# ipo-lab/lqp_py

Hardware: AMD Instinct MI355X
Metric: QPs/sec forward+backward, batch=128 dz=500 tol=1e-5 (higher is better)
Workload: dtype f32; 1 GPU; BASELINE configs[2]: batch=128/GPU dz=500 m=1 box+equality QP, ADMM forward + fixed-point backward, eps 1e-5, scale+adaptive_rho defaults; global_batch=128, seeds=10 batches, seeds 0..9 per rank, cycled, iters=60, checks=4, launch_mode=3, sync=False, linsolve=spd, loop_workgroups_per_qp=2, parallelism=batch-sharded x1, rccl_world_size=1

## Files before the change

### include/lqp_amd.h

```cpp
#ifndef LQP_AMD_H
#define LQP_AMD_H

#include <stddef.h>
#include <stdint.h>

#ifdef __cplusplus
extern "C" {
#endif

#define LQP_ABI_VERSION 14

enum { LQP_F32 = 0, LQP_F64 = 1 };

enum {
    LQP_OK = 0,
    LQP_ERR_INVALID = 1,
    LQP_ERR_WORKSPACE = 2,
    LQP_ERR_SINGULAR = 3,
    LQP_ERR_HIP = 4,
    LQP_ERR_TIMEOUT = 5,
    LQP_ERR_UNSUPPORTED = 6,
    LQP_ERR_NOT_SPD = 7
};

typedef struct lqp_boxqp_ctrl {
    int32_t max_iters;
    int32_t check_solved;
    int32_t adaptive_rho;
    int32_t adaptive_rho_iter;
    int32_t adaptive_rho_max_iter;
    int32_t scale;
    int32_t any_lb;
    int32_t any_ub;
    int32_t rho_mode;
    int32_t beta_mode;
    int32_t launch_mode;
    int32_t reserved;
    int32_t linsolve;
    int32_t reserved2;
    double eps_abs;
    double eps_rel;
    double rho_value;
    double rho_min;
// ... 7 lines not shown
    const void* bound_flags_in;
    void* host_report;
} lqp_boxqp_ctrl;

typedef struct lqp_boxqp_stats {
    int32_t iters;
    int32_t n_factor;
    int32_t n_solve;
    int32_t n_check;
    int32_t rho_updated;
    int32_t fail_index;
    int32_t n_launch;
    int32_t mode_used;
    int32_t linsolve_used;
    int32_t factor_launches;
    int32_t loop_workgroups;
    int32_t any_lb;
    int32_t any_ub;
    int32_t loop_kind;
} lqp_boxqp_stats;

int lqp_abi_version(void);
const char* lqp_status_string(int status);

void lqp_profile_enable(int on);
void lqp_profile_reset(void);
int lqp_profile_classes(void);
const char* lqp_profile_class_name(int cls);
int lqp_profile_get(double* total_ms, long long* launches, int n);
void lqp_debug_set_lu_counters(void* device_buf);
int lqp_debug_spin(void* stream, int blocks, int usec, int lds_bytes);
int lqp_debug_xcd(void* stream, int blocks, void* out_dev);
int lqp_debug_lu_inverse(void* stream, int dtype, int B, int N, const void* packed, void* X_out);

size_t lqp_boxqp_forward_workspace_bytes(int dtype, int B, int n, int m);
int lqp_boxqp_forward_layout(int dtype, int B, int n, int m, size_t* status_offset, size_t* status_bytes,
                             size_t* info_offset, size_t* info_bytes);
int lqp_boxqp_forward(void* stream, int dtype, int B, int n, int m,
                      const void* Q, const void* p, const void* A, const void* b,
                      const void* lb, const void* ub,
                      const lqp_boxqp_ctrl* ctrl, const void* rho_in,
                      void* x, void* z, void* u, void* lams, void* nus, void* rho_out,
                      lqp_boxqp_stats* stats,
                      void* workspace, size_t workspace_bytes);

int lqp_boxqp_forward_finish(void* stream, int B, int max_iters, int check_solved, const void* host_report,
                             lqp_boxqp_stats* stats);

size_t lqp_boxqp_unroll_backward_workspace_bytes(int B, int n, int m, int iters);
int lqp_boxqp_unroll_backward(void* stream, int B, int n, int m, const void* fwd_workspace, size_t fwd_workspace_bytes,
                              int iters, const void* dl_dx, void* dQs, void* dps, void* dAs, void* dbs, void* dlbs,
                              void* dubs, void* drho, void* dD, void* scratch, size_t scratch_bytes);

size_t lqp_boxqp_unroll_backward_lu_workspace_bytes(int dtype, int B, int n, int m, int iters);
int lqp_boxqp_unroll_backward_lu(void* stream, int dtype, int B, int n, int m, const void* fwd_workspace, size_t fwd_workspace_bytes,
                                 int iters, const void* dl_dx, void* dQs, void* dps, void* dAs, void* dbs, void* dlbs, void* dubs,
                                 void* drho, void* dD, void* scratch, size_t scratch_bytes);

size_t lqp_boxqp_unroll_tape_workspace_bytes(int dtype, int B, int n, int m, int iters);
int lqp_boxqp_unroll_tape_segment(void* stream, int dtype, int B, int n, int m, const void* fwd_workspace, size_t fwd_workspace_bytes,
                                  int iters, int k0, int k1, int mode, const void* packed_buf, const void* rho, void* state, int inj_k,
                                  const void* inj, const void* dl_dx, void* dps, void* dlbs, void* dubs, void* drho, void* dD,
                                  void* scratch, size_t scratch_bytes, void** z_rows, void** u_rows, void** x_rows);
int lqp_boxqp_unroll_tape_finish(void* stream, int dtype, int B, int n, int m, int iters, void* dQs, void* dAs, void* dbs, void* scratch,
                                 size_t scratch_bytes);

// ... 79 lines not shown
```

### lqp_py_amd/_lib.py

```python
import ctypes
import os
import subprocess
import threading

import numpy

import torch

HERE = os.path.dirname(os.path.abspath(__file__))
CSRC = os.path.join(HERE, "csrc")
LIB_PATH = os.environ.get("LQP_LIB", os.path.join(CSRC, "liblqp_amd.so"))
SOURCES = ["lqp_amd.hip", "lqp_unroll.hpp", "lqp_boxqp.hpp", "lqp_loop_split.hpp", "lqp_loop_small.hpp", "lqp_lu.hpp", "lqp_lu_big.hpp", "lqp_lu2.hpp", "lqp_lu_wide.hpp", "lqp_dense.hpp", "lqp_trsv.hpp", "lqp_spd.hpp", "lqp_f16x2.hpp", "lqp_common.hpp"]

LQP_F32, LQP_F64 = 0, 1
ABI_VERSION = 14
STATUS = {0: "ok", 1: "invalid argument", 2: "workspace too small", 3: "singular", 4: "HIP error",
          5: "grid barrier timeout", 6: "unsupported size (n + m <= 4096 in float32, 2048 in float64)", 7: "matrix outside the symmetric x-update"}

c_void_p, c_int, c_size_t, c_double = ctypes.c_void_p, ctypes.c_int, ctypes.c_size_t, ctypes.c_double


CHECK_HOOK = ctypes.CFUNCTYPE(ctypes.c_int, ctypes.c_void_p, ctypes.c_void_p, ctypes.c_void_p, ctypes.c_int)


class BoxQPCtrl(ctypes.Structure):
    _fields_ = [(k, ctypes.c_int32) for k in (
        "max_iters", "check_solved", "adaptive_rho", "adaptive_rho_iter", "adaptive_rho_max_iter", "scale",
        "any_lb", "any_ub", "rho_mode", "beta_mode", "launch_mode", "reserved", "linsolve", "reserved2")] + [
        (k, ctypes.c_double) for k in (
            "eps_abs", "eps_rel", "rho_value", "rho_min", "rho_max", "adaptive_rho_tol",
            "adaptive_rho_threshold", "beta_value")] + [
        ("beta_in", ctypes.c_void_p), ("check_hook", CHECK_HOOK), ("check_hook_user", ctypes.c_void_p),
        ("bound_flags_in", ctypes.c_void_p), ("host_report", ctypes.c_void_p)]


class BoxQPStats(ctypes.Structure):
    _fields_ = [(k, ctypes.c_int32) for k in (
        "iters", "n_factor", "n_solve", "n_check", "rho_updated", "fail_index", "n_launch", "mode_used", "linsolve_used",
        "factor_launches", "loop_workgroups", "any_lb", "any_ub", "loop_kind")]


_P = c_void_p
SYMBOLS = {
    "lqp_abi_version": (c_int, []),
    "lqp_status_string": (ctypes.c_char_p, [c_int]),
    "lqp_profile_enable": (None, [c_int]),
    "lqp_profile_reset": (None, []),
    "lqp_profile_classes": (c_int, []),
    "lqp_profile_class_name": (ctypes.c_char_p, [c_int]),
    "lqp_profile_get": (c_int, [ctypes.POINTER(c_double), ctypes.POINTER(ctypes.c_longlong), c_int]),
    "lqp_debug_set_lu_counters": (None, [_P]),
    "lqp_debug_spin": (c_int, [_P, c_int, c_int, c_int]),
    "lqp_debug_xcd": (c_int, [_P, c_int, _P]),
    "lqp_debug_lu_inverse": (c_int, [_P, c_int, c_int, c_int, _P, _P]),
    "lqp_boxqp_forward_workspace_bytes": (c_size_t, [c_int] * 4),
    "lqp_boxqp_forward": (c_int, [_P, c_int, c_int, c_int, c_int, _P, _P, _P, _P, _P, _P,
                                  ctypes.POINTER(BoxQPCtrl), _P, _P, _P, _P, _P, _P, _P,
                                  ctypes.POINTER(BoxQPStats), _P, c_size_t]),
    "lqp_boxqp_forward_finish": (c_int, [_P, c_int, c_int, c_int, _P, ctypes.POINTER(BoxQPStats)]),
    "lqp_boxqp_forward_layout": (c_int, [c_int] * 4 + [ctypes.POINTER(c_size_t)] * 4),
    "lqp_boxqp_unroll_backward_workspace_bytes": (c_size_t, [c_int] * 4),
    "lqp_boxqp_unroll_backward": (c_int, [_P, c_int, c_int, c_int, _P, c_size_t, c_int] + [_P] * 10 + [c_size_t]),
    "lqp_boxqp_unroll_backward_lu_workspace_bytes": (c_size_t, [c_int] * 5),
    "lqp_boxqp_unroll_backward_lu": (c_int, [_P, c_int, c_int, c_int, c_int, _P, c_size_t, c_int] + [_P] * 10 + [c_size_t]),
    "lqp_boxqp_unroll_tape_workspace_bytes": (c_size_t, [c_int] * 5),
    "lqp_boxqp_unroll_tape_segment": (c_int, [_P, c_int, c_int, c_int, c_int, _P, c_size_t, c_int, c_int, c_int, c_int, _P, _P, _P, c_int]
                                      + [_P] * 8 + [c_size_t] + [_P] * 3),
    "lqp_boxqp_unroll_tape_finish": (c_int, [_P, c_int, c_int, c_int, c_int, c_int, _P, _P, _P, _P, c_size_t]),
    "lqp_unroll_scale_colmax": (c_int, [_P, c_int, c_int, _P, _P, _P, _P]),
    "lqp_unroll_scale_grad_slabs": (c_int, [c_int, c_int]),
    "lqp_unroll_scale_grad": (c_int, [_P, c_int, c_int, _P, _P, _P, _P, _P, c_int]),
    "lqp_unroll_scale_vectors": (c_int, [_P, c_int, c_int, c_int, c_int, c_int, c_int, c_double] + [_P] * 13 + [c_int] + [_P] * 7),
    "lqp_unroll_scale_scatter": (c_int, [_P, c_int, c_int, _P, _P, _P, _P, _P, _P]),
    "lqp_boxqp_last_residuals": (c_int, [_P, c_int, c_int, c_int, c_int, _P, c_size_t, _P, _P]),
    "lqp_boxqp_problem_iters": (c_int, [_P, c_int, c_int, c_int, c_int, _P, c_size_t, _P]),
    "lqp_boxqp_check_trace": (c_int, [_P, c_int, c_int, c_int, c_int, _P, c_size_t, c_int, _P]),
    "lqp_boxqp_backward_fp_workspace_bytes": (c_size_t, [c_int] * 4),
    "lqp_boxqp_backward_fp_prefactor": (c_int, [_P, c_int, c_int, c_int, c_int] + [_P] * 6 + [_P, c_size_t, c_int, _P]),
    "lqp_boxqp_backward_fp": (c_int, [_P, c_int, c_int, c_int, c_int] + [_P] * 9 + [c_int, c_double, _P] + [_P] * 6 +
                              [ctypes.POINTER(ctypes.c_int32), _P, c_size_t, c_int, _P]),
    "lqp_boxqp_backward_kkt": (c_int, [_P, c_int, c_int, c_int, c_int] + [_P] * 8 + [_P] * 6 +
                               [ctypes.POINTER(ctypes.c_int32), _P, c_size_t, c_int, _P]),
    "lqp_lu_factor_workspace_bytes": (c_size_t, [c_int] * 3),
    "lqp_lu_factor_batched": (c_int, [_P, c_int, c_int, c_int, _P, _P, _P, _P, c_size_t]),
    "lqp_lu_solve_workspace_bytes": (c_size_t, [c_int] * 3),
    "lqp_lu_solve_batched": (c_int, [_P, c_int, c_int, c_int, c_int, _P, _P, _P, _P, c_size_t]),
    "lqp_lu_packed_bytes": (c_size_t, [c_int] * 3),
# ... 315 lines not shown
```

### lqp_py_amd/csrc/lqp_amd.hip

```cpp
#include "../../include/lqp_amd.h"
#include "lqp_boxqp.hpp"
#include "lqp_unroll.hpp"
#ifdef LQP_SPLIT_BUILD
#include "split/lqp_extern.inc"
#endif

#include <cstdio>
#include <cstdlib>
#include <cstring>
#include <algorithm>
#include <atomic>
#include <chrono>
#include <mutex>
#include <vector>
#include <string>
#include <type_traits>
#include <unordered_map>
#include <unordered_set>

using namespace lqp;

namespace {

constexpr int kRing = 2048;
// ... 1740 lines not shown
    smem[threadIdx.x] = 0;
    const unsigned long long t0 = __builtin_amdgcn_s_memrealtime();
    while (__builtin_amdgcn_s_memrealtime() - t0 < ticks) __builtin_amdgcn_s_sleep(32);
}
int lqp_debug_spin(void* stream, int blocks, int usec, int lds_bytes) {
    if (blocks < 1 || usec < 0 || usec > 2000000 || lds_bytes < 512) return LQP_ERR_INVALID;
    const int rc = ensure_lds((const void*)k_debug_spin, lds_bytes);
    if (rc) return rc;
    hipLaunchKernelGGL(k_debug_spin, dim3(blocks), dim3(512), lds_bytes, (hipStream_t)stream, (unsigned long long)usec * 100ull);
    return last_error();
}

__global__ __launch_bounds__(512) void k_debug_xcd(int* __restrict__ out) {
    if (threadIdx.x == 0) out[blockIdx.x] = (int)my_xcd();
}
int lqp_debug_xcd(void* stream, int blocks, void* out_dev) {
    if (blocks < 1 || !out_dev) return LQP_ERR_INVALID;
    hipLaunchKernelGGL(k_debug_xcd, dim3(blocks), dim3(512), 0, (hipStream_t)stream, (int*)out_dev);
    return last_error();
}

int lqp_debug_lu_inverse(void* stream, int dtype, int B, int N, const void* packed_buf, void* X_out) {
    if (bad_dims(dtype, B, N, 0) || !packed_buf || !X_out || N > (dtype == LQP_F32 ? 2048 : 1024)) return LQP_ERR_INVALID;
    const int K = round_up(N, LQP_NB) / LQP_NB;
    return by_dtype(dtype, [&](auto t) {
        using T = decltype(t);
        int* dest; T* packed;
        carve_packed<T>((void*)packed_buf, B, N, dest, packed);
        return launch_lu_inverse<T>((hipStream_t)stream, B, N, packed, packed_blocks(K) * LQP_BLK, dest, K * LQP_NB, (T*)X_out,
                                    (size_t)N * N, N, nullptr);
    });
}

int lqp_profile_classes(void) { return PC_COUNT; }

const char* lqp_profile_class_name(int c) {
    static const char* names[PC_COUNT] = {"fwd_setup", "lu_factor", "pack", "admm_loop", "rho_update", "fwd_epilogue",
                                          "bwd_build", "packed_solve", "bwd_epilogue", "misc", "admm_loop_tail",
                                          "spd_inverse", "eq_correct", "bwd_cholesky", "unroll_backward", "unroll_scaling"};
    return (c >= 0 && c < PC_COUNT) ? names[c] : "?";
}

int lqp_profile_get(double* total_ms, long long* launches, int n) {
    std::lock_guard<std::mutex> lock(g_prof_mutex);
    for (auto& r : g_prof_recs) {
        if (hipEventSynchronize(r.b) != hipSuccess) return LQP_ERR_HIP;
        float ms = 0.f;
        if (hipEventElapsedTime(&ms, r.a, r.b) != hipSuccess) return LQP_ERR_HIP;
        g_prof_ms[r.cls] += ms;
        g_prof_n[r.cls] += 1;
        (void)hipEventDestroy(r.a); (void)hipEventDestroy(r.b);
    }
    g_prof_recs.clear();
    for (int i = 0; i < n && i < PC_COUNT; ++i) { total_ms[i] = g_prof_ms[i]; launches[i] = g_prof_n[i]; }
    return LQP_OK;
}

const char* lqp_status_string(int s) {
    switch (s) {
        case LQP_OK: return "ok";
        case LQP_ERR_INVALID: return "invalid argument";
        case LQP_ERR_WORKSPACE: return "workspace too small";
        case LQP_ERR_SINGULAR: return "singular matrix (exactly zero pivot)";
        case LQP_ERR_HIP: return "HIP runtime error";
        case LQP_ERR_TIMEOUT: return "in-kernel grid barrier timed out";
        case LQP_ERR_UNSUPPORTED: return "size not supported by this build (n + m <= 4096 in float32, 2048 in float64)";
// ... 391 lines not shown
```

### lqp_py_amd/csrc/lqp_boxqp.hpp

```cpp
#pragma once
#include <type_traits>
#include "lqp_common.hpp"
#include "lqp_lu.hpp"
#include "lqp_lu_big.hpp"
#include "lqp_lu2.hpp"
#include "lqp_lu_wide.hpp"
#include "lqp_trsv.hpp"
#include "lqp_spd.hpp"

namespace lqp {

enum { ST_DONE = 0, ST_FINAL_ITER = 1, ST_GATE = 2, ST_NFACTOR = 3, ST_RHO_UPDATED = 4,
       ST_TIMEOUT = 5, ST_NCHECK = 6, ST_NOTSPD = 7,
       ST_VOTE = 8,
       ST_ANY_LB = 12, ST_ANY_UB = 13,
       ST_RESUME = 14,
       ST_NDONE = 15,
       ST_WORDS = 16 };
enum { PS_DONE = 0, PS_FINAL = 1, PS_RESUME = 2, PS_NFACTOR = 3, PS_WORDS = 4 };
enum { RP_LB = 1, RP_UB = 2, RP_TIMEOUT = 4, RP_NOTSPD = 8 };
enum { CT_NOTOPT = 0, CT_ARRIVE = 1, CT_WANTS = 2, CT_TRIG = 3, CT_WORDS = 4 };
template <typename T>
__device__ __forceinline__ void trace_check(unsigned int* __restrict__ vtrace, const int it, const int check_solved, const int ring,
                                            const T pri, const T dua) {
// ... 2035 lines not shown
    extern __shared__ __attribute__((aligned(32))) char smem[];
    const int b = blockIdx.x, n = P.n, m = P.m, Np = P.Np;
    const int tid = threadIdx.x, lane = tid & 63, w = tid >> 6;
    const int Kmax = round_up(n, LQP_NB) / LQP_NB, Npm = Kmax * LQP_NB;
    const int nf = P.nred[b] - m;
    const int Kb = round_up(nf, LQP_NB) / LQP_NB, Nb = Kb * LQP_NB;
    float* Ls = P.packed + (size_t)b * sym_blocks(Kmax) * LQP_BLK;
    const float* AF = P.M + (size_t)b * Np * Np;
    float* rhs = P.rhs + (size_t)b * Np;
    unsigned long long dt0 = P.dbg ? clock64() : 0;
    if (Kb > 0 && P.phase != 2) {
        if (Kb <= P.la_maxk) wg_chol_factor_la<F16>(Ls, Kb, P.info + b, smem, P.dbg ? P.dbg + (size_t)b * 8 : nullptr);
        else if (Kb <= SPD_MAXK) wg_chol_factor(Ls, Kb, P.info + b, smem);
        else wg_chol_factor_big(Ls, Kb, P.info + b, smem);
    }
    if (P.host_report && (P.early_report || P.phase == 1) && !P.reported) {
        __syncthreads();
        if (tid == 0)
            __hip_atomic_store(P.host_report + b, __hip_atomic_load(P.info + b, __ATOMIC_RELAXED, __HIP_MEMORY_SCOPE_AGENT),
                               __ATOMIC_RELAXED, __HIP_MEMORY_SCOPE_SYSTEM);
    }
    if (P.phase == 1) return;
    __syncthreads();
    if (P.dbg && tid == 0) { const unsigned long long t = clock64(); P.dbg[(size_t)b * 8 + 0] = t - dt0; dt0 = t; P.dbg[(size_t)b * 8 + 3] = Kb; }
    constexpr int NR = NRV == 4 ? 4 : 2;
    float* acc = (float*)smem;
    float* u0 = acc + (size_t)NR * Npm;
    float* G = u0 + Npm;
    float* t = G + (size_t)m * Npm;
    float* part = t + NR * 64;
    float* S = part + NR * LQP_NW * 64;
    float* wv = S + m * m;
    float* dn = wv + m;
    if (P.phase == 2) {
        const float* g = P.g + (size_t)b * n;
        const int* fidx = P.fidx + (size_t)b * n;
        const float* bs_ = P.bsc ? P.bsc + (size_t)b * Np : nullptr;
        for (int e = tid; e < Nb; e += LQP_NT) u0[e] = e < nf ? -g[fidx[e]] * (bs_ ? bs_[e] : 1.f) : 0.f;
    } else {
        for (int e = tid; e < Nb; e += LQP_NT) u0[e] = rhs[e];
    }
    for (int q = 0; q < m; ++q)
        for (int e = tid; e < Nb; e += LQP_NT) G[(size_t)q * Npm + e] = AF[(size_t)q * Npm + e];
    __syncthreads();
    if (Kb > 0)
        for (int c0 = 0; c0 < 1 + m; c0 += NR)
            wg_chol_solve_n<NR>(Ls, Kb, u0 + (size_t)c0 * Npm, Npm, (1 + m - c0) < NR ? (1 + m - c0) : NR, acc, t, part,
                                (P.dbg && P.la_maxk == 0) ? P.dbg + (size_t)b * 8 : nullptr);
    if (P.dbg && tid == 0) { const unsigned long long t = clock64(); P.dbg[(size_t)b * 8 + 1] = t - dt0; dt0 = t; }
    if (m > 0) {
        for (int e = w; e < m * m + m; e += LQP_NW) {
            const int q = e < m * m ? e / m : e - m * m;
            const float* rv = e < m * m ? G + (size_t)(e - q * m) * Npm : u0;
            float a = 0.f;
            for (int i = lane; i < nf; i += 64) a += AF[(size_t)q * Npm + i] * rv[i];
            a = wave_sum(a);
            if (lane == 0) {
                if (e < m * m) S[e] = a - ((e / m == e % m) ? 1e-8f : 0.f);
                else wv[q] = a;
            }
        }
        __syncthreads();
        {
            const int rr = tid / (m + 1), jj = tid - rr * (m + 1);
            const bool mine = tid < m * (m + 1);
            int* pivrow = (int*)dn;
            for (int c = 0; c < m; ++c) {
                if (tid == 0) {
                    int pr = c;
                    float best = tabs(S[c * m + c]);
                    for (int r2 = c + 1; r2 < m; ++r2) if (tabs(S[r2 * m + c]) > best) { best = tabs(S[r2 * m + c]); pr = r2; }
                    const bool skip = !(best > 0.f);
                    if (skip && P.info[b] == 0) P.info[b] = nf + c + 1;
                    pivrow[0] = pr; pivrow[1] = skip ? 1 : 0;
                }
                __syncthreads();
                const int pr = pivrow[0];
                const bool skip = pivrow[1] != 0;
                float* const rowc = jj < m ? S + c * m + jj : wv + c;
                float* const rowp = jj < m ? S + pr * m + jj : wv + pr;
                float* const rowr = jj < m ? S + rr * m + jj : wv + rr;
                if (!skip && pr != c && tid <= m) {
                    const float tmp = *rowc; *rowc = *rowp; *rowp = tmp;
                }
                __syncthreads();
                const float inv = skip ? 0.f : 1.f / S[c * m + c];
                const float f = (mine && !skip) ? S[rr * m + c] : 0.f;
                __syncthreads();
                if (!skip && tid <= m) *rowc *= inv;
                __syncthreads();
                if (mine && !skip && rr != c) *rowr -= f * *rowc;
                __syncthreads();
            }
            for (int q = tid; q < m; q += LQP_NT) dn[q] = wv[q];
        }
        __syncthreads();
    }
    for (int a = tid; a < nf; a += LQP_NT) {
        float d = u0[a];
        for (int q = 0; q < m; ++q) d -= G[(size_t)q * Npm + a] * dn[q];
        rhs[a] = P.bsc ? d * P.bsc[(size_t)b * Np + a] : d;
    }
    for (int q = tid; q < m; q += LQP_NT) rhs[nf + q] = dn[q];
    if (P.dbg && tid == 0) P.dbg[(size_t)b * 8 + 2] = clock64() - dt0;
}

template <typename T>
__global__ __launch_bounds__(LQP_NT) void k_bwd_residual(const BwdParams<T> P) {
    extern __shared__ __attribute__((aligned(32))) char smem[];
    const int b = blockIdx.x, n = P.n, m = P.m, Np = P.Np;
    const int tid = threadIdx.x, lane = tid & 63, w = tid >> 6;
    T* dvf = (T*)smem;
    T* dn = dvf + round_up(n, 8);
    int* fl = (int*)(dn + round_up(m > 0 ? m : 1, 8));
    const int nf = P.nred[b] - m;
    const T* d = P.rhs + (size_t)b * Np;
    T* r = P.rhs2 + (size_t)b * Np;
    const T* Q = P.Q + (size_t)b * n * n;
    const T* A = P.A ? P.A + (size_t)b * m * n : nullptr;
    const T* g = P.g + (size_t)b * n;
    for (int i = tid; i < n; i += LQP_NT) dvf[i] = T(0);
    for (int a = tid; a < nf; a += LQP_NT) fl[a] = P.fidx[(size_t)b * n + a];
    for (int q = tid; q < m; q += LQP_NT) dn[q] = d[nf + q];
    __syncthreads();
    for (int a = tid; a < nf; a += LQP_NT) dvf[fl[a]] = d[a];
    __syncthreads();
    constexpr int RG = 4;
    const int ny = (int)gridDim.y, me = (int)blockIdx.y;
    for (int a0 = (w * ny + me) * RG; a0 < nf + m; a0 += LQP_NW * ny * RG) {
        const T* row[RG];
        double acc[RG];
#pragma unroll
        for (int u = 0; u < RG; ++u) {
            const int a = min(a0 + u, nf + m - 1);
            row[u] = a >= nf ? A + (size_t)(a - nf) * n : Q + (size_t)fl[a] * n;
            acc[u] = 0.0;
        }
// ... 252 lines not shown
```

### lqp_py_amd/csrc/lqp_spd.hpp

```cpp
#pragma once
#include "lqp_common.hpp"
#include "lqp_lu.hpp"
#include "lqp_trsv.hpp"
#include "lqp_f16x2.hpp"

namespace lqp {

constexpr int SPD_LS = 68;
constexpr int SPD_MAXK = 8;
constexpr int SPD_MAXM = 16;

__host__ __device__ constexpr int sym_blocks(int K) { return K * (K + 1) / 2; }
__host__ __device__ constexpr int sym_idx(int i, int j, int K) { return j * K - j * (j - 1) / 2 + (i - j); }
#ifndef LQP_PIV_WAVES
#define LQP_PIV_WAVES 16
#endif
#ifndef LQP_PIV_WAVES_RS
#define LQP_PIV_WAVES_RS 8
#endif
#ifndef LQP_PIV_NB
#define LQP_PIV_NB 4
#endif
constexpr int PIV_NB = LQP_PIV_NB;
constexpr int PIV_LDS = 2 * PIV_NB * 64 + 64;
// ... 2952 lines not shown
                }
            }
        }
#pragma unroll
        for (int c = 0; c < NR; ++c) fold(a2[c], c);
        __syncthreads();
        if (tc < nc) {
            float sum = 0.f;
#pragma unroll
            for (int ww = 0; ww < LQP_NW; ++ww) sum += part[((size_t)tc * LQP_NW + ww) * 64 + te];
            t[tc * 64 + te] = X[(size_t)tc * xs + j * 64 + te] - sum;
        }
        __syncthreads();
#pragma unroll
        for (int c = 0; c < NR; ++c) {
            const float tr = t[c * 64 + r];
#pragma unroll
            for (int e = 0; e < 4; ++e) a2[c][e] = bd.v[e] * tr;
            fold(a2[c], c);
        }
        if (j > 0) bd = blk4(j - 1, j - 1);
        __syncthreads();
        if (tc < nc) {
            float sum = 0.f;
#pragma unroll
            for (int ww = 0; ww < LQP_NW; ++ww) sum += part[((size_t)tc * LQP_NW + ww) * 64 + te];
            X[(size_t)tc * xs + j * 64 + te] = sum;
        }
        __syncthreads();
    }
    if (dbg && threadIdx.x == 0) dbg[5] += clock64() - c0;
}

}
```

### lqp_py_amd/csrc/split/lqp_extern.inc

```
extern template __global__ void lqp::k_bwd_chol_solve<0, true>(lqp::BwdParams<float>);
extern template __global__ void lqp::k_bwd_chol_solve<4, true>(lqp::BwdParams<float>);
extern template __global__ void lqp::k_spd_resident<8, 2, true>(lqp::FwdParams<float>, int const*);
extern template __global__ void lqp::k_spd_resident<5, 2, true>(lqp::FwdParams<float>, int const*);
extern template __global__ void lqp::k_spd_resident<6, 2, true>(lqp::FwdParams<float>, int const*);
extern template __global__ void lqp::k_spd_resident<7, 2, true>(lqp::FwdParams<float>, int const*);
extern template __global__ void lqp::k_spd_resident<3, 2, true>(lqp::FwdParams<float>, int const*);
extern template __global__ void lqp::k_spd_resident<4, 2, true>(lqp::FwdParams<float>, int const*);
extern template __global__ void lqp::k_spd_resident<7, 4, true>(lqp::FwdParams<float>, int const*);
extern template __global__ void lqp::k_spd_resident<8, 4, true>(lqp::FwdParams<float>, int const*);
extern template __global__ void lqp::k_spd_resident<3, 2, false>(lqp::FwdParams<float>, int const*);
extern template __global__ void lqp::k_spd_resident<4, 2, false>(lqp::FwdParams<float>, int const*);
extern template __global__ void lqp::k_spd_resident<5, 2, false>(lqp::FwdParams<float>, int const*);
extern template __global__ void lqp::k_spd_resident<6, 2, false>(lqp::FwdParams<float>, int const*);
extern template __global__ void lqp::k_spd_resident<7, 2, false>(lqp::FwdParams<float>, int const*);
extern template __global__ void lqp::k_spd_resident<7, 4, false>(lqp::FwdParams<float>, int const*);
extern template __global__ void lqp::k_spd_resident<8, 2, false>(lqp::FwdParams<float>, int const*);
extern template __global__ void lqp::k_spd_resident<8, 4, false>(lqp::FwdParams<float>, int const*);
extern template __global__ void lqp::k_admm_loop_split<3, 512, false, 2>(lqp::FwdParams<float>, int, int, int);
extern template __global__ void lqp::k_admm_loop_split<4, 512, false, 2>(lqp::FwdParams<float>, int, int, int);
extern template __global__ void lqp::k_admm_loop_split<5, 512, false, 2>(lqp::FwdParams<float>, int, int, int);
extern template __global__ void lqp::k_admm_loop_split<6, 512, false, 2>(lqp::FwdParams<float>, int, int, int);
extern template __global__ void lqp::k_admm_loop_split<7, 512, false, 2>(lqp::FwdParams<float>, int, int, int);
extern template __global__ void lqp::k_admm_loop_split<7, 512, false, 4>(lqp::FwdParams<float>, int, int, int);
extern template __global__ void lqp::k_admm_loop_split<8, 512, false, 2>(lqp::FwdParams<float>, int, int, int);
// ... 24 lines not shown
extern template __global__ void lqp::k_admm_loop<float, true, false, 1024, false>(lqp::FwdParams<float>, int, int, int, int, int);
extern template __global__ void lqp::k_admm_loop<float, true, false, 1024, true>(lqp::FwdParams<float>, int, int, int, int, int);
extern template __global__ void lqp::k_admm_loop<float, true, false, 512, false>(lqp::FwdParams<float>, int, int, int, int, int);
extern template __global__ void lqp::k_admm_loop<float, true, false, 512, true>(lqp::FwdParams<float>, int, int, int, int, int);
extern template __global__ void lqp::k_admm_loop_dense<double>(lqp::FwdParams<double>, int, int, int);
extern template __global__ void lqp::k_admm_loop_dense<float>(lqp::FwdParams<float>, int, int, int);
extern template __global__ void lqp::k_admm_loop_dense_w<double>(lqp::FwdParams<double>, int, int, int, int);
extern template __global__ void lqp::k_admm_loop_dense_w<float>(lqp::FwdParams<float>, int, int, int, int);
extern template __global__ void lqp::k_lu_inverse<double, false>(double const*, unsigned long, int, int, int const*, int, double*, unsigned long, int, int const*);
extern template __global__ void lqp::k_lu_inverse<float, false>(float const*, unsigned long, int, int, int const*, int, float*, unsigned long, int, int const*);
extern template __global__ void lqp::k_lu_inverse<float, true>(float const*, unsigned long, int, int, int const*, int, float*, unsigned long, int, int const*);
extern template __global__ void lqp::k_lu_factor2<double, 16>(double*, int, int, unsigned long, int*, int, int*, int const*, int const*, unsigned long long*, unsigned long, unsigned int, unsigned long long*, int, int);
extern template __global__ void lqp::k_lu_factor2<float, 32>(float*, int, int, unsigned long, int*, int, int*, int const*, int const*, unsigned long long*, unsigned long, unsigned int, unsigned long long*, int, int);
extern template __global__ void lqp::k_lu_factor<float, 16, true, 1024>(float*, int, int, unsigned long, int*, int, int*, int const*, unsigned long long*, int const*);
extern template __global__ void lqp::k_lu_factor<float, 16, true, 512>(float*, int, int, unsigned long, int*, int, int*, int const*, unsigned long long*, int const*);
extern template __global__ void lqp::k_lu_factor<float, 32, true, 512>(float*, int, int, unsigned long, int*, int, int*, int const*, unsigned long long*, int const*);
extern template __global__ void lqp::k_lu_factor_big<double>(double*, int, int, unsigned long, int*, int, int*, int const*, int const*);
extern template __global__ void lqp::k_lu_factor_big<float>(float*, int, int, unsigned long, int*, int, int*, int const*, int const*);
extern template __global__ void lqp::k_lu_factor_wide<double>(double*, int, int, unsigned long, int*, int, int*, int const*, int const*, int*, unsigned long, unsigned int, int, unsigned long long*);
extern template __global__ void lqp::k_lu_factor_wide<float>(float*, int, int, unsigned long, int*, int, int*, int const*, int const*, int*, unsigned long, unsigned int, int, unsigned long long*);
extern template __global__ void lqp::k_lu_factor_wide_tall<float>(float*, int, int, unsigned long, int*, int, int*, int const*, int const*, int*, unsigned long, unsigned int, int, unsigned long long*);
extern template __global__ void lqp::k_lu_factor<double, 16, true, 1024>(double*, int, int, unsigned long, int*, int, int*, int const*, unsigned long long*, int const*);
extern template __global__ void lqp::k_lu_factor<double, 16, true, 512>(double*, int, int, unsigned long, int*, int, int*, int const*, unsigned long long*, int const*);
extern template __global__ void lqp::k_lu_factor<double, 8, true, 1024>(double*, int, int, unsigned long, int*, int, int*, int const*, unsigned long long*, int const*);
extern template __global__ void lqp::k_lu_factor<double, 8, true, 512>(double*, int, int, unsigned long, int*, int, int*, int const*, unsigned long long*, int const*);
extern template __global__ void lqp::k_lu_factor<float, 16, false, 1024>(float*, int, int, unsigned long, int*, int, int*, int const*, unsigned long long*, int const*);
extern template __global__ void lqp::k_lu_factor<float, 16, false, 512>(float*, int, int, unsigned long, int*, int, int*, int const*, unsigned long long*, int const*);
extern template __global__ void lqp::k_lu_factor<float, 32, false, 512>(float*, int, int, unsigned long, int*, int, int*, int const*, unsigned long long*, int const*);
extern template __global__ void lqp::k_lu_factor<float, 8, false, 1024>(float*, int, int, unsigned long, int*, int, int*, int const*, unsigned long long*, int const*);
extern template __global__ void lqp::k_lu_factor<float, 8, false, 512>(float*, int, int, unsigned long, int*, int, int*, int const*, unsigned long long*, int const*);
extern template __global__ void lqp::k_bwd_build_chol<0>(lqp::BwdParams<float>);
extern template __global__ void lqp::k_bwd_chol_solve<0, false>(lqp::BwdParams<float>);
extern template __global__ void lqp::k_bwd_chol_solve<4, false>(lqp::BwdParams<float>);
extern template __global__ void lqp::k_spd_begin<0>(lqp::FwdParams<float>, int const*);
extern template __global__ void lqp::k_spd_big_step<0>(lqp::FwdParams<float>, int const*, int, int);
extern template __global__ void lqp::k_spd_end<0>(lqp::FwdParams<float>, int const*);
extern template __global__ void lqp::k_spd_inverse<1>(lqp::FwdParams<float>, int const*);
extern template __global__ void lqp::k_spd_inverse<2>(lqp::FwdParams<float>, int const*);
extern template __global__ void lqp::k_spd_inverse_dense<1>(float const*, float*, float*, int*, int, int, float*);
extern template __global__ void lqp::k_spd_inverse_dense<2>(float const*, float*, float*, int*, int, int, float*);
extern template __global__ void lqp::k_spd_prep<0>(lqp::FwdParams<float>);
extern template __global__ void lqp::k_spd_rho_big<0>(lqp::FwdParams<float>);
extern template __global__ void lqp::k_spd_step<0>(lqp::FwdParams<float>, int const*, int, int);
extern template __global__ void lqp::k_admm_loop_small<0>(lqp::FwdParams<float>, int, int, int);
extern template __global__ void lqp::k_unroll_lu_eq<double>(lqp::UnrollLuParams<double>, int, int);
extern template __global__ void lqp::k_unroll_lu_eq<float>(lqp::UnrollLuParams<float>, int, int);
extern template __global__ void lqp::k_unroll_outer<0>(float const*, float const*, float*, int, int);
extern template __global__ void lqp::k_unroll_outer_any<double>(double const*, double const*, double*, int, int);
extern template __global__ void lqp::k_unroll_outer_any<float>(float const*, float const*, float*, int, int);
extern template __global__ void lqp::k_unroll_scale_colmax<0>(float const*, int, float*, int*, int*);
extern template __global__ void lqp::k_unroll_scale_grad<0>(float const*, float const*, float const*, float*, int, float*);
extern template __global__ void lqp::k_unroll_scale_scatter<0>(float const*, float const*, int const*, int const*, float const*, float*, int);
extern template __global__ void lqp::k_unroll_scale_vectors<0>(lqp::ScaleVecParams);
extern template __global__ void lqp::k_unroll_sweep<16>(lqp::FwdParams<float>, lqp::UnrollParams);
extern template __global__ void lqp::k_unroll_sweep<1>(lqp::FwdParams<float>, lqp::UnrollParams);
extern template __global__ void lqp::k_unroll_sweep_lu<double>(lqp::FwdParams<double>, lqp::UnrollLuParams<double>);
extern template __global__ void lqp::k_unroll_sweep_lu<float>(lqp::FwdParams<float>, lqp::UnrollLuParams<float>);
extern template __global__ void lqp::k_unroll_sweep_split<5, 16>(lqp::FwdParams<float>, lqp::UnrollParams, unsigned int);
extern template __global__ void lqp::k_unroll_sweep_split<6, 16>(lqp::FwdParams<float>, lqp::UnrollParams, unsigned int);
extern template __global__ void lqp::k_unroll_sweep_split<7, 16>(lqp::FwdParams<float>, lqp::UnrollParams, unsigned int);
extern template __global__ void lqp::k_unroll_sweep_split<8, 16>(lqp::FwdParams<float>, lqp::UnrollParams, unsigned int);
extern template __global__ void lqp::k_unroll_sweep_split<8, 1>(lqp::FwdParams<float>, lqp::UnrollParams, unsigned int);
extern template __global__ void lqp::k_admm_loop_np2<0>(lqp::FwdParams<float>, int, int, int, int, int);
extern template __global__ void lqp::k_admm_loop_small_each<0>(lqp::FwdParams<float>, int, int, int);
extern template __global__ void lqp::k_bwd_build<double>(lqp::BwdParams<double>);
extern template __global__ void lqp::k_bwd_build<float>(lqp::BwdParams<float>);
// ... 34 lines not shown
```

### lqp_py_amd/csrc/split/lqp_tu_spd.hip

```cpp
#include "../lqp_unroll.hpp"
template __global__ void lqp::k_bwd_build_chol<0>(lqp::BwdParams<float>);
template __global__ void lqp::k_bwd_chol_solve<0, false>(lqp::BwdParams<float>);
template __global__ void lqp::k_bwd_chol_solve<4, false>(lqp::BwdParams<float>);
template __global__ void lqp::k_spd_begin<0>(lqp::FwdParams<float>, int const*);
template __global__ void lqp::k_spd_big_step<0>(lqp::FwdParams<float>, int const*, int, int);
template __global__ void lqp::k_spd_end<0>(lqp::FwdParams<float>, int const*);
template __global__ void lqp::k_spd_inverse<1>(lqp::FwdParams<float>, int const*);
template __global__ void lqp::k_spd_inverse<2>(lqp::FwdParams<float>, int const*);
template __global__ void lqp::k_spd_inverse_dense<1>(float const*, float*, float*, int*, int, int, float*);
template __global__ void lqp::k_spd_inverse_dense<2>(float const*, float*, float*, int*, int, int, float*);
template __global__ void lqp::k_spd_prep<0>(lqp::FwdParams<float>);
template __global__ void lqp::k_spd_rho_big<0>(lqp::FwdParams<float>);
template __global__ void lqp::k_spd_step<0>(lqp::FwdParams<float>, int const*, int, int);
```

Baseline: 202,800 QPs/sec.

## Keep Cholesky factor blocks in registers for small backward triangular solves

Adds a register-resident Cholesky solve path that is used when the factor has at most 4 or 6 blocks of 64. Factor blocks are loaded once into VGPRs and reused across all right-hand-side rounds instead of being re-read from global memory or LDS. This replaces the generic wg_chol_solve_n in the backward solve and fuses the RHS fill before the loads. It also adds a debug kernel for testing the solve. The cost is higher register pressure, and the path only triggers for small free-set sizes.

```diff
diff --git a/include/lqp_amd.h b/include/lqp_amd.h
--- a/include/lqp_amd.h
+++ b/include/lqp_amd.h
@@ -8,7 +8,7 @@
 extern "C" {
 #endif
 
-#define LQP_ABI_VERSION 14
+#define LQP_ABI_VERSION 15
 
 enum { LQP_F32 = 0, LQP_F64 = 1 };
 
@@ -82,6 +82,8 @@
 int lqp_debug_spin(void* stream, int blocks, int usec, int lds_bytes);
 int lqp_debug_xcd(void* stream, int blocks, void* out_dev);
 int lqp_debug_lu_inverse(void* stream, int dtype, int B, int N, const void* packed, void* X_out);
+int lqp_debug_chol_solve(void* stream, int B, int Kmax, const void* packed, const void* kb, int nrhs, int nr, int which,
+                         const void* V, void* X_out);
 
 size_t lqp_boxqp_forward_workspace_bytes(int dtype, int B, int n, int m);
 int lqp_boxqp_forward_layout(int dtype, int B, int n, int m, size_t* status_offset, size_t* status_bytes,
diff --git a/lqp_py_amd/_lib.py b/lqp_py_amd/_lib.py
--- a/lqp_py_amd/_lib.py
+++ b/lqp_py_amd/_lib.py
@@ -13,7 +13,7 @@
 SOURCES = ["lqp_amd.hip", "lqp_unroll.hpp", "lqp_boxqp.hpp", "lqp_loop_split.hpp", "lqp_loop_small.hpp", "lqp_lu.hpp", "lqp_lu_big.hpp", "lqp_lu2.hpp", "lqp_lu_wide.hpp", "lqp_dense.hpp", "lqp_trsv.hpp", "lqp_spd.hpp", "lqp_f16x2.hpp", "lqp_common.hpp"]
 
 LQP_F32, LQP_F64 = 0, 1
-ABI_VERSION = 14
+ABI_VERSION = 15
 STATUS = {0: "ok", 1: "invalid argument", 2: "workspace too small", 3: "singular", 4: "HIP error",
           5: "grid barrier timeout", 6: "unsupported size (n + m <= 4096 in float32, 2048 in float64)", 7: "matrix outside the symmetric x-update"}
 
@@ -53,6 +53,7 @@
     "lqp_debug_spin": (c_int, [_P, c_int, c_int, c_int]),
     "lqp_debug_xcd": (c_int, [_P, c_int, _P]),
     "lqp_debug_lu_inverse": (c_int, [_P, c_int, c_int, c_int, _P, _P]),
+    "lqp_debug_chol_solve": (c_int, [_P, c_int, c_int, _P, _P, c_int, c_int, c_int, _P, _P]),
     "lqp_boxqp_forward_workspace_bytes": (c_size_t, [c_int] * 4),
     "lqp_boxqp_forward": (c_int, [_P, c_int, c_int, c_int, c_int, _P, _P, _P, _P, _P, _P,
                                   ctypes.POINTER(BoxQPCtrl), _P, _P, _P, _P, _P, _P, _P,
diff --git a/lqp_py_amd/csrc/lqp_amd.hip b/lqp_py_amd/csrc/lqp_amd.hip
--- a/lqp_py_amd/csrc/lqp_amd.hip
+++ b/lqp_py_amd/csrc/lqp_amd.hip
@@ -1796,6 +1796,19 @@
     });
 }
 
+int lqp_debug_chol_solve(void* stream, int B, int Kmax, const void* packed, const void* kb, int nrhs, int nr, int which,
+                         const void* V, void* X_out) {
+    if (B < 1 || Kmax < 1 || Kmax > SPD_MAXK || nrhs < 1 || nrhs > 32 || (nr != 2 && nr != 4) || (which != 0 && which != 1) ||
+        !packed || !kb || !V || !X_out) return LQP_ERR_INVALID;
+    const int lds = debug_chol_solve_lds_bytes(Kmax, nrhs, nr);
+    auto fn = nr == 4 ? k_debug_chol_solve<4> : k_debug_chol_solve<2>;
+    const int rc = ensure_lds((const void*)fn, lds);
+    if (rc) return rc;
+    hipLaunchKernelGGL(fn, dim3(B), dim3(LQP_NT), lds, (hipStream_t)stream, (const float*)packed, (const int*)kb, (const float*)V,
+                       (float*)X_out, Kmax, nrhs, which);
+    return last_error();
+}
+
 int lqp_profile_classes(void) { return PC_COUNT; }
 
 const char* lqp_profile_class_name(int c) {
diff --git a/lqp_py_amd/csrc/lqp_boxqp.hpp b/lqp_py_amd/csrc/lqp_boxqp.hpp
--- a/lqp_py_amd/csrc/lqp_boxqp.hpp
+++ b/lqp_py_amd/csrc/lqp_boxqp.hpp
@@ -2091,21 +2091,23 @@
     float* S = part + NR * LQP_NW * 64;
     float* wv = S + m * m;
     float* dn = wv + m;
-    if (P.phase == 2) {
-        const float* g = P.g + (size_t)b * n;
-        const int* fidx = P.fidx + (size_t)b * n;
-        const float* bs_ = P.bsc ? P.bsc + (size_t)b * Np : nullptr;
-        for (int e = tid; e < Nb; e += LQP_NT) u0[e] = e < nf ? -g[fidx[e]] * (bs_ ? bs_[e] : 1.f) : 0.f;
-    } else {
-        for (int e = tid; e < Nb; e += LQP_NT) u0[e] = rhs[e];
-    }
-    for (int q = 0; q < m; ++q)
-        for (int e = tid; e < Nb; e += LQP_NT) G[(size_t)q * Npm + e] = AF[(size_t)q * Npm + e];
-    __syncthreads();
-    if (Kb > 0)
-        for (int c0 = 0; c0 < 1 + m; c0 += NR)
-            wg_chol_solve_n<NR>(Ls, Kb, u0 + (size_t)c0 * Npm, Npm, (1 + m - c0) < NR ? (1 + m - c0) : NR, acc, t, part,
-                                (P.dbg && P.la_maxk == 0) ? P.dbg + (size_t)b * 8 : nullptr);
+    auto fill = [&]() {
+        if (P.phase == 2) {
+            const float* g = P.g + (size_t)b * n;
+            const int* fidx = P.fidx + (size_t)b * n;
+            const float* bs_ = P.bsc ? P.bsc + (size_t)b * Np : nullptr;
+#pragma unroll 1
+            for (int e = tid; e < Nb; e += LQP_NT) u0[e] = e < nf ? -g[fidx[e]] * (bs_ ? bs_[e] : 1.f) : 0.f;
+        } else {
+#pragma unroll 1
+            for (int e = tid; e < Nb; e += LQP_NT) u0[e] = rhs[e];
+        }
+        for (int q = 0; q < m; ++q)
+#pragma unroll 1
+            for (int e = tid; e < Nb; e += LQP_NT) G[(size_t)q * Npm + e] = AF[(size_t)q * Npm + e];
+    };
+    wg_chol_solve_all<NR>(Ls, Kb, u0, Npm, 1 + m, acc, t, part, true, fill,
+                          (P.dbg && P.la_maxk == 0) ? P.dbg + (size_t)b * 8 : nullptr);
     if (P.dbg && tid == 0) { const unsigned long long t = clock64(); P.dbg[(size_t)b * 8 + 1] = t - dt0; dt0 = t; }
     if (m > 0) {
         for (int e = w; e < m * m + m; e += LQP_NW) {
@@ -2162,6 +2164,32 @@
     }
     for (int q = tid; q < m; q += LQP_NT) rhs[nf + q] = dn[q];
     if (P.dbg && tid == 0) P.dbg[(size_t)b * 8 + 2] = clock64() - dt0;
+}
+
+__host__ __device__ inline int debug_chol_solve_lds_bytes(int Kmax, int nrhs, int nr) {
+    return ((nr + nrhs) * Kmax * LQP_NB + nr * 64 + nr * LQP_NW * 64) * 4;
+}
+template <int NR>
+__global__ __launch_bounds__(LQP_NT) void k_debug_chol_solve(const float* __restrict__ packed, const int* __restrict__ kb,
+                                                             const float* __restrict__ V, float* __restrict__ Xo, const int Kmax,
+                                                             const int nrhs, const int reg) {
+    extern __shared__ __attribute__((aligned(32))) char smem[];
+    const int b = blockIdx.x, tid = threadIdx.x, Npm = Kmax * LQP_NB;
+    const int K = min(max(kb[b], 0), Kmax), Nb = K * LQP_NB;
+    const float* Ls = packed + (size_t)b * sym_blocks(Kmax) * LQP_BLK;
+    const float* Vb = V + (size_t)b * nrhs * Npm;
+    float* Xb = Xo + (size_t)b * nrhs * Npm;
+    float* acc = (float*)smem;
+    float* X = acc + (size_t)NR * Npm;
+    float* t = X + (size_t)nrhs * Npm;
+    float* part = t + NR * 64;
+    auto fill = [&]() {
+        for (int c = 0; c < nrhs; ++c)
+            for (int e = tid; e < Nb; e += LQP_NT) X[(size_t)c * Npm + e] = Vb[(size_t)c * Npm + e];
+    };
+    wg_chol_solve_all<NR>(Ls, K, X, Npm, nrhs, acc, t, part, reg != 0, fill);
+    for (int c = 0; c < nrhs; ++c)
+        for (int e = tid; e < Npm; e += LQP_NT) Xb[(size_t)c * Npm + e] = e < Nb ? X[(size_t)c * Npm + e] : 0.f;
 }
 
 template <typename T>
diff --git a/lqp_py_amd/csrc/lqp_spd.hpp b/lqp_py_amd/csrc/lqp_spd.hpp
--- a/lqp_py_amd/csrc/lqp_spd.hpp
+++ b/lqp_py_amd/csrc/lqp_spd.hpp
@@ -3008,4 +3008,192 @@
     if (dbg && threadIdx.x == 0) dbg[5] += clock64() - c0;
 }
 
-}
+#ifndef LQP_CHOL_SOLVE_REG
+#define LQP_CHOL_SOLVE_REG 1
+#endif
+template <int NR> constexpr int chol_reg_maxk() { return NR > 2 ? 4 : 6; }
+template <int NR> constexpr int chol_reg_blocks() { return NR > 2 ? 10 : 15; }
+template <int V> struct IntC { static constexpr int value = V; };
+template <int NB> struct CholRegs { V4<float> b[NB]; };
+__device__ __forceinline__ V4<float> chol_blk_load(const float* __restrict__ Ls, const int q) {
+    return *(const V4<float>*)(Ls + (size_t)q * LQP_BLK + threadIdx.x * 4);
+}
+__device__ __forceinline__ V4<float> chol_blk_reload(const float* __restrict__ Ls, int q) {
+    asm volatile("" : "+s"(q));
+    return chol_blk_load(Ls, q);
+}
+template <int NB>
+__device__ __forceinline__ void chol_regs_load(const float* __restrict__ Ls, const int K, CholRegs<NB>& R) {
+    const int nblk = sym_blocks(K);
+#pragma unroll
+    for (int q = 0; q < NB; ++q)
+        if (q < nblk) R.b[q] = chol_blk_load(Ls, q);
+}
+
+__device__ __forceinline__ float chol_dot4(const V4<float>& a, const V4<float>& b) {
+    return __builtin_fmaf(a.v[3], b.v[3], __builtin_fmaf(a.v[2], b.v[2], __builtin_fmaf(a.v[0], b.v[0], a.v[1] * b.v[1])));
+}
+
+template <int K, int NR, int NB>
+__device__ __forceinline__ void wg_chol_solve_reg(const float* __restrict__ Ls, CholRegs<NB>& R, float* __restrict__ X,
+                                                  const int xs, const int nc, float* __restrict__ t, float* __restrict__ part,
+                                                  unsigned long long* __restrict__ dbg = nullptr) {
+    constexpr bool SHARE = sym_blocks(K) > NB;
+    constexpr int NSH = SHARE ? sym_blocks(K) - NB : 0;
+    static_assert(!SHARE || (NSH == K && sym_idx(3, 3, K) == NB), "the shared form: K = 6 on 15 resident blocks");
+    unsigned long long c0 = dbg ? clock64() : 0;
+    const int tid = threadIdx.x, r = tid >> 4, cq = tid & 15, lane = tid & 63, w = tid >> 6;
+    const int tc = tid >> 6, te = tid & 63;
+    auto blk = [&](const int i, const int j) -> const V4<float>& {
+        const int q = sym_idx(i, j, K);
+        return R.b[q < NB ? q : q - NB];
+    };
+    float acc[NR][K];
+    float yl[NR];
+#pragma unroll
+    for (int c = 0; c < NR; ++c) {
+        yl[c] = 0.f;
+#pragma unroll
+        for (int i = 0; i < K; ++i) acc[c][i] = 0.f;
+    }
+    if (cq == 0) {
+#pragma unroll
+        for (int c = 0; c < NR; ++c)
+            if (c < nc) t[c * 64 + r] = X[(size_t)c * xs + r] - acc[c][0];
+    }
+    wg_barrier_lds();
+#pragma unroll
+    for (int j = 0; j < K; ++j) {
+#pragma unroll
+        for (int c = 0; c < NR; ++c) {
+            if (c < nc) {
+                const float s1 = rowgroup_sum<LQP_NT>(chol_dot4(blk(j, j), *(const V4<float>*)(t + c * 64 + cq * 4)));
+                if (j + 1 < K) { if (cq == 0) X[(size_t)c * xs + j * 64 + r] = s1; }
+                else yl[c] = __int_as_float(__builtin_amdgcn_ds_bpermute((lane & 48) << 2, __float_as_int(s1)));
+            }
+        }
+        if (j + 1 < K) {
+            wg_barrier_lds();
+            V4<float> yj[NR];
+#pragma unroll
+            for (int c = 0; c < NR; ++c) yj[c] = *(const V4<float>*)(X + (size_t)(c < nc ? c : 0) * xs + j * 64 + cq * 4);
+#pragma unroll
+            for (int i = j + 1; i < K; ++i) {
+#pragma unroll
+                for (int c = 0; c < NR; ++c)
+                    if (c < nc) acc[c][i] += rowgroup_sum<LQP_NT>(chol_dot4(blk(i, j), yj[c]));
+            }
+            if constexpr (SHARE) {
+                if (j == 0) {
+#pragma unroll
+                    for (int q = 0; q < NSH; ++q) R.b[q] = chol_blk_reload(Ls, NB + q);
+                }
+            }
+            if (cq == 0) {
+#pragma unroll
+                for (int c = 0; c < NR; ++c)
+                    if (c < nc) t[c * 64 + r] = X[(size_t)c * xs + (j + 1) * 64 + r] - acc[c][j + 1];
+            }
+            wg_barrier_lds();
+        }
+    }
+    auto fold = [&](float (&a2)[4], const int c) {
+        col_fold<4>(a2);
+        part[((size_t)c * LQP_NW + w) * 64 + cq * 4 + col_fold_elem(lane)] = a2[0];
+    };
+    if (dbg && threadIdx.x == 0) { const unsigned long long c1 = clock64(); dbg[4] += c1 - c0; c0 = c1; }
+#pragma unroll
+    for (int j = K - 1; j >= 0; --j) {
+        if constexpr (SHARE) {
+            if (j == 2) {
+#pragma unroll
+                for (int q = 0; q < NSH; ++q) R.b[q] = chol_blk_reload(Ls, q);
+            }
+        }
+        float a2[NR][4];
+        float tr[NR];
+        if (j + 1 < K) {
+#pragma unroll
+            for (int c = 0; c < NR; ++c)
+#pragma unroll
+                for (int e = 0; e < 4; ++e) a2[c][e] = 0.f;
+#pragma unroll
+            for (int i = j + 1; i < K; ++i) {
+#pragma unroll
+                for (int c = 0; c < NR; ++c) {
+                    const float xi = X[(size_t)(c < nc ? c : 0) * xs + i * 64 + r];
+#pragma unroll
+                    for (int e = 0; e < 4; ++e) a2[c][e] = __builtin_fmaf(blk(i, j).v[e], xi, a2[c][e]);
+                }
+            }
+#pragma unroll
+            for (int c = 0; c < NR; ++c) fold(a2[c], c);
+            wg_barrier_lds();
+            if (tc < nc) {
+                float sum = 0.f;
+#pragma unroll
+                for (int ww = 0; ww < LQP_NW; ++ww) sum += part[((size_t)tc * LQP_NW + ww) * 64 + te];
+                t[tc * 64 + te] = X[(size_t)tc * xs + j * 64 + te] - sum;
+            }
+            wg_barrier_lds();
+#pragma unroll
+            for (int c = 0; c < NR; ++c) tr[c] = t[c * 64 + r];
+        } else {
+#pragma unroll
+            for (int c = 0; c < NR; ++c) tr[c] = yl[c];
+        }
+#pragma unroll
+        for (int c = 0; c < NR; ++c) {
+#pragma unroll
+            for (int e = 0; e < 4; ++e) a2[c][e] = blk(j, j).v[e] * tr[c];
+            fold(a2[c], c);
+        }
+        wg_barrier_lds();
+        if (tc < nc) {
+            float sum = 0.f;
+#pragma unroll
+            for (int ww = 0; ww < LQP_NW; ++ww) sum += part[((size_t)tc * LQP_NW + ww) * 64 + te];
+            X[(size_t)tc * xs + j * 64 + te] = sum;
+        }
+        wg_barrier_lds();
+    }
+    if (dbg && threadIdx.x == 0) dbg[5] += clock64() - c0;
+}
+
+template <int NR, typename Fill>
+__device__ __forceinline__ void wg_chol_solve_all(const float* __restrict__ Ls, const int K, float* __restrict__ X, const int xs,
+                                                  const int ntot, float* __restrict__ acc, float* __restrict__ t,
+                                                  float* __restrict__ part, const bool reg, Fill&& fill,
+                                                  unsigned long long* __restrict__ dbg = nullptr) {
+    auto rounds = [&](auto&& solve) {
+        for (int c0 = 0; c0 < ntot; c0 += NR) solve(X + (size_t)c0 * xs, (ntot - c0) < NR ? (ntot - c0) : NR);
+    };
+#if LQP_CHOL_SOLVE_REG
+    constexpr int MAXK = chol_reg_maxk<NR>(), NB = chol_reg_blocks<NR>();
+    if (reg && K >= 1 && K <= MAXK) {
+        fill();
+        CholRegs<NB> R;
+        chol_regs_load<NB>(Ls, K, R);
+        wg_barrier_lds();
+        auto run = [&](auto kc) {
+            constexpr int KC = decltype(kc)::value;
+            if constexpr (KC <= MAXK)
+                rounds([&](float* Xc, const int nc) { wg_chol_solve_reg<KC, NR, NB>(Ls, R, Xc, xs, nc, t, part, dbg); });
+        };
+        switch (K) {
+            case 1: run(IntC<1>{}); break;
+            case 2: run(IntC<2>{}); break;
+            case 3: run(IntC<3>{}); break;
+            case 4: run(IntC<4>{}); break;
+            case 5: run(IntC<5>{}); break;
+            default: run(IntC<6>{}); break;
+        }
+        return;
+    }
+#endif
+    fill();
+    __syncthreads();
+    if (K > 0) rounds([&](float* Xc, const int nc) { wg_chol_solve_n<NR>(Ls, K, Xc, xs, nc, acc, t, part, dbg); });
+}
+
+}
diff --git a/lqp_py_amd/csrc/split/lqp_extern.inc b/lqp_py_amd/csrc/split/lqp_extern.inc
--- a/lqp_py_amd/csrc/split/lqp_extern.inc
+++ b/lqp_py_amd/csrc/split/lqp_extern.inc
@@ -80,6 +80,8 @@
 extern template __global__ void lqp::k_bwd_build_chol<0>(lqp::BwdParams<float>);
 extern template __global__ void lqp::k_bwd_chol_solve<0, false>(lqp::BwdParams<float>);
 extern template __global__ void lqp::k_bwd_chol_solve<4, false>(lqp::BwdParams<float>);
+extern template __global__ void lqp::k_debug_chol_solve<2>(float const*, int const*, float const*, float*, int, int, int);
+extern template __global__ void lqp::k_debug_chol_solve<4>(float const*, int const*, float const*, float*, int, int, int);
 extern template __global__ void lqp::k_spd_begin<0>(lqp::FwdParams<float>, int const*);
 extern template __global__ void lqp::k_spd_big_step<0>(lqp::FwdParams<float>, int const*, int, int);
 extern template __global__ void lqp::k_spd_end<0>(lqp::FwdParams<float>, int const*);
diff --git a/lqp_py_amd/csrc/split/lqp_tu_spd.hip b/lqp_py_amd/csrc/split/lqp_tu_spd.hip
--- a/lqp_py_amd/csrc/split/lqp_tu_spd.hip
+++ b/lqp_py_amd/csrc/split/lqp_tu_spd.hip
@@ -2,6 +2,8 @@
 template __global__ void lqp::k_bwd_build_chol<0>(lqp::BwdParams<float>);
 template __global__ void lqp::k_bwd_chol_solve<0, false>(lqp::BwdParams<float>);
 template __global__ void lqp::k_bwd_chol_solve<4, false>(lqp::BwdParams<float>);
+template __global__ void lqp::k_debug_chol_solve<2>(float const*, int const*, float const*, float*, int, int, int);
+template __global__ void lqp::k_debug_chol_solve<4>(float const*, int const*, float const*, float*, int, int, int);
 template __global__ void lqp::k_spd_begin<0>(lqp::FwdParams<float>, int const*);
 template __global__ void lqp::k_spd_big_step<0>(lqp::FwdParams<float>, int const*, int, int);
 template __global__ void lqp::k_spd_end<0>(lqp::FwdParams<float>, int const*);
```

New measurement: 205,400 QPs/sec, median of 6. 1.01x the previous value.
